# microsoft/fadtk

Measured on AMD Instinct MI355X. Metric: FAD scores/sec + cov-GEMM TFLOP/s (% MFMA peak), N=100k D=512, higher is better.
Workload: dtype f16 in, f16 MFMA with f32 accumulate over <= 8192-row runs, f64 across runs (moments); split-f16 MFMA iterations (f32 accumulate) + exact int8-MFMA products (int32 accumulate) + f64 correction (Frechet)

## Files before the change

### fadtk_amd/csrc/frechet.hip

```cpp
#include "frechet_internal.h"
#include "ns_mean.h"
#include "ns_fast.h"
#include "ns_fast_big.h"
#include "ns_fast_res.h"

#include <algorithm>
#include <atomic>
#include <cmath>
#include <type_traits>

namespace fad {

Pool& thread_pool(int device) {
    static thread_local PerThreadDevice<Pool> set;
    return set.get(device);
}
Workspace* free_slot(int device) {
    Pool& p = thread_pool(device);
    for (Workspace& w : p.slot)
        if (!w.busy) { w.pool = &p; return &w; }
    return nullptr;
}

SongKnobs SongKnobs::from_env() {
// ... 201 lines not shown
    }
    return f;
}

static int fast_prepare(Workspace& ws, int d, int ddof, const double* acc1, const double* acc2, const double* cov1, const double* cov2,
                        const double* mu1, const double* mu2, int mean_dtype, double* mus, double* covs, hipStream_t st,
                        const float* run1 = nullptr, const float* run2 = nullptr) {
    void* const before = ws.fast.p;
    FAD_TRY(ws.fast.reserve(fast_bytes(d)));
    FAD_TRY(ws.small.reserve(ns_small_bytes(d, 1)));
    FastBufs f = fast_bufs(ws, d);
    if (ws.fast.p != before) FAD_HIP_TRY(hipMemsetAsync(f.hdr, 0, 256, st));
    ws.job.gen = ++ws.fast_gen;
    if (ws.fast_gen > (1 << 30)) ws.fast_gen = 1;
    nsf::PrepArgs a;
    memset(&a, 0, sizeof(a));
    a.acc[0] = acc1; a.acc[1] = acc2; a.cov_in[0] = cov1; a.cov_in[1] = cov2; a.mu_in[0] = mu1; a.mu_in[1] = mu2;
    a.run[0] = run1; a.run[1] = run2;
    a.d = d; a.ddof = ddof; a.gen = ws.job.gen; a.mean_dtype = mean_dtype;
    a.mus = mus; a.covs = covs;
    a.dig[0] = f.digC[0]; a.dig[1] = f.digC[1];
    a.st = static_cast<NsState*>(ws.small.p);
    a.hdr[0] = f.hdr; a.hdr[1] = f.hdr + 1;
    hipLaunchKernelGGL(nsf::nsf_prepare, dim3((unsigned)((int64_t)d * d / 2048 + 1), 2), dim3(512), 0, st, a);
    FAD_HIP_TRY(hipGetLastError());
    return FAD_OK;
}

template <int NS> static void fast_launch_split(int mode, unsigned t, unsigned B, const nsf::SplitArgs& g, hipStream_t st) {
    if (mode == nsf::SP_FIRST) hipLaunchKernelGGL((nsf::nsf_split<NS, nsf::SP_FIRST>), dim3(t, t, B), dim3(512), 0, st, g);
    else if (mode == nsf::SP_T) hipLaunchKernelGGL((nsf::nsf_split<NS, nsf::SP_T>), dim3(t, t, B), dim3(512), 0, st, g);
    else if (mode == nsf::SP_V2) hipLaunchKernelGGL((nsf::nsf_split<NS, nsf::SP_V2>), dim3(t, t, 2 * B), dim3(512), 0, st, g);
    else if (mode == nsf::SP_V3) hipLaunchKernelGGL((nsf::nsf_split<NS, nsf::SP_V3>), dim3(t, t, B), dim3(512), 0, st, g);
    else hipLaunchKernelGGL((nsf::nsf_split<NS, nsf::SP_U>), dim3(t, t, 3 * B), dim3(512), 0, st, g);
}
static void fast_split(int d, int mode, const nsf::SplitArgs& g, hipStream_t st, unsigned B);
static void fast_verify_launch(int d, unsigned B, nsf::SplitArgs g, const nsf::SplitMat (&Y)[2], const nsf::SplitMat (&Z)[2], const nsf::SplitMat& Rv,
                               const nsf::SplitMat& Pv, const nsf::SplitMat& Ev, const Ns32State* s32, double* vstats, int* vwords, int64_t hstride,
                               hipStream_t st) {
    g.sel = &s32->final_iter; g.skip = &s32->skip_corr;
    g.Zf[0] = Z[0]; g.Zf[1] = Z[1]; g.Yf[0] = Y[0]; g.Yf[1] = Y[1];
    g.vstats = vstats; g.vwords = vwords; g.hstride = hstride;
    g.B[0] = Rv; g.C[0] = Pv; g.C[1] = Ev;
    fast_split(d, nsf::SP_V2, g, st, B);
    g.B[0] = Pv; g.A[1] = Ev; g.C[0] = nsf::SplitMat{nullptr, nullptr}; g.C[1] = nsf::SplitMat{nullptr, nullptr};
    fast_split(d, nsf::SP_V3, g, st, B);
}
static void fast_split(int d, int mode, const nsf::SplitArgs& g, hipStream_t st, unsigned B) {
    const unsigned t = (unsigned)(d / 32);
    switch (d) {
        case 128: fast_launch_split<1>(mode, t, B, g, st); break;
        case 256: fast_launch_split<2>(mode, t, B, g, st); break;
        case 384: fast_launch_split<3>(mode, t, B, g, st); break;
        case 512: fast_launch_split<4>(mode, t, B, g, st); break;
        case 768: fast_launch_split<6>(mode, t, B, g, st); break;
        default: fast_launch_split<8>(mode, t, B, g, st); break;
    }
}
template <int NJ> static void fast_big_attrs() {
    (void)hipFuncSetAttribute(reinterpret_cast<const void*>(&nsf::nsf_big<nsf::SP_T, NJ>), hipFuncAttributeMaxDynamicSharedMemorySize, (int)nsf::kBigLds);
    (void)hipFuncSetAttribute(reinterpret_cast<const void*>(&nsf::nsf_big<nsf::SP_U, NJ>), hipFuncAttributeMaxDynamicSharedMemorySize, (int)nsf::kBigLds);
    (void)hipFuncSetAttribute(reinterpret_cast<const void*>(&nsf::nsf_big<nsf::SP_FIRST, NJ>), hipFuncAttributeMaxDynamicSharedMemorySize, (int)nsf::kBigLds);
}
template <int NJ> static void fast_big_launch(int d, int mode, const nsf::SplitArgs& g, hipStream_t st, unsigned B) {
    const int tt = nsf::big_tiles(d, NJ);
    const unsigned one = (unsigned)nsf::big_grid((int)B, tt), two = (unsigned)nsf::big_grid((int)B, 2 * tt);
    if (mode == nsf::SP_FIRST) hipLaunchKernelGGL((nsf::nsf_big<nsf::SP_FIRST, NJ>), dim3(one), dim3(256), nsf::kBigLds, st, g);
    else if (mode == nsf::SP_T) hipLaunchKernelGGL((nsf::nsf_big<nsf::SP_T, NJ>), dim3(one), dim3(256), nsf::kBigLds, st, g);
    else hipLaunchKernelGGL((nsf::nsf_big<nsf::SP_U, NJ>), dim3(two + B), dim3(256), nsf::kBigLds, st, g);
}
static int fast_big_t_slots(int d, unsigned B) { return nsf::big_tiles(d, nsf::big_nj(d, 1, (int)B)); }
static int fast_split_big(int d, int mode, nsf::SplitArgs g, hipStream_t st, unsigned B, int device) {
    static std::atomic<unsigned> ready{0};
    if (device >= 0 && device < 32 && !(ready.load(std::memory_order_acquire) & (1u << device))) {
        fast_big_attrs<1>(); fast_big_attrs<2>();
        FAD_HIP_TRY(hipGetLastError());
        ready.fetch_or(1u << device, std::memory_order_release);
    }
    g.nprob = (int)B;
    if (nsf::big_nj(d, mode == nsf::SP_U ? 2 : 1, (int)B) == 1) fast_big_launch<1>(d, mode, g, st, B);
    else fast_big_launch<2>(d, mode, g, st, B);
    return FAD_OK;
}
static int fast_i8_big(int d, int mode, const nsf::I8Args& g, hipStream_t st, unsigned B, int device) {
    static std::atomic<unsigned> ready{0};
    if (device >= 0 && device < 32 && !(ready.load(std::memory_order_acquire) & (1u << device))) {
        FAD_HIP_TRY(hipFuncSetAttribute(reinterpret_cast<const void*>(&nsf::nsf_i8_big<nsf::I8_A>), hipFuncAttributeMaxDynamicSharedMemorySize, (int)nsf::kI8BigLds));
        FAD_HIP_TRY(hipFuncSetAttribute(reinterpret_cast<const void*>(&nsf::nsf_i8_big<nsf::I8_G>), hipFuncAttributeMaxDynamicSharedMemorySize, (int)nsf::kI8BigLds));
        FAD_HIP_TRY(hipFuncSetAttribute(reinterpret_cast<const void*>(&nsf::nsf_i8_big<nsf::I8_G, true>), hipFuncAttributeMaxDynamicSharedMemorySize, (int)nsf::kI8BigLds));
        ready.fetch_or(1u << device, std::memory_order_release);
    }
    const unsigned grid = (unsigned)nsf::big_grid((int)B, (d / 128) * (d / 64));
    if (mode == nsf::I8_A) hipLaunchKernelGGL((nsf::nsf_i8_big<nsf::I8_A>), dim3(grid), dim3(512), nsf::kI8BigLds, st, g, (int)B);
    else if (g.Rv.a) hipLaunchKernelGGL((nsf::nsf_i8_big<nsf::I8_G, true>), dim3(grid), dim3(512), nsf::kI8BigLds, st, g, (int)B);
    else hipLaunchKernelGGL((nsf::nsf_i8_big<nsf::I8_G>), dim3(grid), dim3(512), nsf::kI8BigLds, st, g, (int)B);
    return FAD_OK;
}
template <int NS8> static void fast_launch_i8(int mode, unsigned t, unsigned B, const nsf::I8Args& g, hipStream_t st) {
    if (mode == nsf::I8_A) hipLaunchKernelGGL((nsf::nsf_i8<NS8, nsf::I8_A>), dim3(t, t, B), dim3(512), 0, st, g);
    else hipLaunchKernelGGL((nsf::nsf_i8<NS8, nsf::I8_G>), dim3(t, t, B), dim3(512), 0, st, g);
}
static void fast_i8(int d, int mode, const nsf::I8Args& g, hipStream_t st, unsigned B = 1) {
    const unsigned t = (unsigned)(d / 32);
    switch (d) {
        case 128: case 256: fast_launch_i8<1>(mode, t, B, g, st); break;
        case 384: case 512: fast_launch_i8<2>(mode, t, B, g, st); break;
        case 768: fast_launch_i8<3>(mode, t, B, g, st); break;
        default: fast_launch_i8<4>(mode, t, B, g, st); break;
    }
}

static nsf::SplitArgs fast_split_args(Workspace& ws, const MixedBufs& m, const FastBufs& f, int d) {
    nsf::SplitArgs g;
    memset(&g, 0, sizeof(g));
    g.d = d; g.gen = ws.job.gen; g.hA = f.hdr; g.hB = f.hdr + 1; g.st = m.dstate; g.s32 = m.s32;
    if (wide_enabled(ws.pool)) { g.scaled = 1; g.lp_wide = 1; g.l0_scale = kWideL0Scale; g.l0_min = kWideL0Min; }
    return g;
}
static int fast_verify_enqueue(Workspace& ws) {
    const int d = ws.job.d;
    MixedBufs m = mixed_bufs(ws, d);
    FastBufs f = fast_bufs(ws, d);
    f.host_words[13] = 0;
    fast_verify_launch(d, 1, fast_split_args(ws, m, f, d), f.Y, f.Z, f.Rv, f.Pv, f.Ev, m.s32, f.host_vstats, f.host_words, 0, ws.job.stream);
    FAD_HIP_TRY(hipGetLastError());
    FAD_HIP_TRY(hipEventRecord(ws.done_ev, ws.job.stream));
    return FAD_OK;
}
static int fast_enqueue(Workspace& ws, int upto) {
    const int d = ws.job.d;
    hipStream_t stream = ws.job.stream;
    MixedBufs m = mixed_bufs(ws, d);
    FastBufs f = fast_bufs(ws, d);
    if (!f.host_words) return set_error(FAD_ERR_ALLOC, "pinned result area of the fast Frechet chain is missing");
    const int nslots = (d / 32) * (d / 32);
    const int max_low = max_low_of(ws);
    for (int& k = ws.job.k; k < upto; ++k) {
        nsf::SplitArgs g = fast_split_args(ws, m, f, d);
        if (k == 0) {
            nsf::I8Args a;
            memset(&a, 0, sizeof(a));
            a.Adig = f.digC[0]; a.Bdig = f.digC[1]; a.d = d; a.gen = ws.job.gen; a.hA = f.hdr; a.hB = f.hdr + 1; a.stats = m.tilestats;
            a.A64 = m.A; a.P = f.P; a.st = m.dstate;
            fast_i8(d, nsf::I8_A, a, stream);
            g.A[0] = f.P; g.B[0] = f.P; g.C[0] = f.Y[1]; g.C[1] = f.Z[1]; g.Cdig[0] = f.digY[1]; g.Cdig_t[0] = f.digYt[1];
            g.A64 = m.A; g.statsA = m.tilestats;
            fast_split(d, nsf::SP_FIRST, g, stream, 1);
            continue;
        }
        const int cur = k & 1;
        g.A[0] = f.Z[cur]; g.B[0] = f.Y[cur]; g.C[0] = f.T; g.alpha = -0.5f; g.beta_eye = 1.5f; g.gamma = 1.0f;
        g.partials = m.partials; g.skip = &m.s32->done; g.k = k;
        fast_split(d, nsf::SP_T, g, stream, 1);
        g = fast_split_args(ws, m, f, d);
        g.A[0] = f.Y[cur]; g.B[0] = f.T; g.C[0] = f.Y[cur ^ 1];
        g.A[1] = f.T; g.B[1] = f.Z[cur]; g.C[1] = f.Z[cur ^ 1];
        g.Cdig[0] = f.digY[cur ^ 1]; g.Cdig_t[0] = f.digYt[cur ^ 1];
        g.skip = &m.s32->upd_skip[k & 1];
        g.k = k; g.max_low = max_low; g.nslots = nslots; g.chk_partials = m.partials;
        g.thr_pred = pred_threshold(ws.pool, d);
        fast_split(d, nsf::SP_U, g, stream, 1);
    }
    nsf::I8Args a;
    memset(&a, 0, sizeof(a));
    a.Adig = f.digY[0]; a.Bdig = f.digYt[0]; a.Adig_alt = f.digY[1]; a.Bdig_alt = f.digYt[1]; a.sel = &m.s32->final_iter;
    a.d = d; a.gen = ws.job.gen; a.hA = f.hdr; a.hB = f.hdr + 1; a.skip = &m.s32->skip_corr; a.stats = f.host_stats; a.st = m.dstate; a.A64in = m.A;
    a.Y[0] = f.Y[0]; a.Y[1] = f.Y[1]; a.Z[0] = f.Z[0]; a.Z[1] = f.Z[1];
    a.s32 = m.s32; a.host_words = f.host_words; a.host_vals = f.host_vals;
    const bool wide = wide_enabled(ws.pool);
    if (wide) { a.Rv = f.Rv; a.scaled = 1; }
    f.host_words[12] = 0;
    f.host_words[13] = 0;
    fast_i8(d, nsf::I8_G, a, stream);
// ... 305 lines not shown
    const int nb = d / 32;
    int* h_words = reinterpret_cast<int*>(hpin + (nsf::kHostVals + (size_t)(nsf::kTileStats + 2) * nb * nb) * sizeof(double));
    double* h_vstats = reinterpret_cast<double*>(hpin + host_vstats_off(d));
    for (int b = 0; b < B; ++b) reinterpret_cast<int*>(reinterpret_cast<char*>(h_words) + (size_t)b * hs)[13] = 0;
    fast_verify_launch(d, (unsigned)B, g, Y, Z, mat(L.Rv), mat(L.Pv), mat(L.Ev), g.s32, h_vstats, h_words, (int64_t)hs, st);
    FAD_HIP_TRY(hipGetLastError());
    FAD_HIP_TRY(hipEventRecord(ws.done_ev, st));
    return FAD_OK;
}

static int pairs_enqueue(Workspace& ws, int d, int B, const fad_moments_t* const* h1, const fad_moments_t* const* h2, int ddof,
                         int mean_dtype, hipStream_t st) {
    const size_t dd = (size_t)d * d;
    const int nb = d / 32;
    constexpr int kPairsBigMin = 3;
    const bool big = B >= kPairsBigMin && d >= 256;
    const bool wide = wide_enabled(ws.pool);
    const int max_low = wide ? kMaxLowWide : kMaxLow;
    const int device = ws.job.device;
    const PairBlock L = pair_block(d);
    const size_t hs = song_host_stride(d);
    void* const before = ws.fast_pairs.p;
    FAD_TRY(ws.fast_pairs.reserve((size_t)(B > 16 ? kMaxMultiPairs : B > 8 ? 16 : B > 4 ? 8 : 4) * L.stride + 256));
    if (!ws.fast_pairs_pin || ws.fast_pairs_pin_cap < (size_t)B * hs) {
        if (ws.fast_pairs_pin) (void)hipHostFree(ws.fast_pairs_pin);
        ws.fast_pairs_pin = nullptr; ws.fast_pairs_pin_cap = 0;
        FAD_HIP_TRY(hipHostMalloc(&ws.fast_pairs_pin, (size_t)kMaxMultiPairs * hs + 4096, hipHostMallocDefault));
        ws.fast_pairs_pin_cap = (size_t)kMaxMultiPairs * hs + 4096;
    }
    char* blk = static_cast<char*>(ws.fast_pairs.p);
    char* hpin = static_cast<char*>(ws.fast_pairs_pin);
    double* h_vals = reinterpret_cast<double*>(hpin);
    double* h_stats = h_vals + nsf::kHostVals;
    int* h_words = reinterpret_cast<int*>(h_stats + (size_t)(nsf::kTileStats + 2) * nb * nb);
    auto at = [&](size_t off) { return blk + off; };
    auto mat = [&](size_t off) { nsf::SplitMat m; m.a = reinterpret_cast<uint4*>(at(off)); m.at = reinterpret_cast<uint4*>(at(off + 4 * dd)); return m; };
    const int gen = ++ws.fast_gen;
    if (ws.fast_gen > (1 << 30)) ws.fast_gen = 1;
    ws.multi.gen = gen;
    if (ws.fast_pairs.p != before) {
        FAD_HIP_TRY(hipMemset2DAsync(at(L.hdrA), L.stride, 0, sizeof(nsf::MatHdr), (size_t)B, st));
        FAD_HIP_TRY(hipMemset2DAsync(at(L.hdrB), L.stride, 0, sizeof(nsf::MatHdr), (size_t)B, st));
    }
    nsf::MatHdr* hA = reinterpret_cast<nsf::MatHdr*>(at(L.hdrA));
    nsf::MatHdr* hB = reinterpret_cast<nsf::MatHdr*>(at(L.hdrB));
    NsState* st0 = reinterpret_cast<NsState*>(at(L.st));
    Ns32State* s32_0 = reinterpret_cast<Ns32State*>(at(L.s32));
    double* partials = reinterpret_cast<double*>(at(L.partials));
    double* stats = reinterpret_cast<double*>(at(L.stats));
    double* A64 = reinterpret_cast<double*>(at(L.A64));
    const nsf::SplitMat P = mat(L.P), Y[2] = {mat(L.Y[0]), mat(L.Y[1])}, Z[2] = {mat(L.Z[0]), mat(L.Z[1])}, T = mat(L.T);
    uint4* digY[2] = {reinterpret_cast<uint4*>(at(L.digY[0])), reinterpret_cast<uint4*>(at(L.digY[1]))};
    uint4* digYt[2] = {reinterpret_cast<uint4*>(at(L.digYt[0])), reinterpret_cast<uint4*>(at(L.digYt[1]))};

    static_assert(2 * kMaxMultiPairs <= nsf::kPrepMaxSets, "PrepArgs holds two sets per pair of a batch");
    nsf::PrepArgs pa;
    memset(&pa, 0, sizeof(pa));
    for (int b = 0; b < B; ++b) {
        pa.accs[2 * b] = moments_packed(h1[b]); pa.accs[2 * b + 1] = moments_packed(h2[b]);
        pa.runs[2 * b] = moments_runsum(h1[b]); pa.runs[2 * b + 1] = moments_runsum(h2[b]);
    }
    pa.acc[0] = pa.accs[0]; pa.acc[1] = pa.accs[1];
    pa.d = d; pa.ddof = ddof; pa.gen = gen; pa.mean_dtype = mean_dtype;
    pa.mus = reinterpret_cast<double*>(at(L.mus)); pa.covs = reinterpret_cast<double*>(at(L.covs));
    pa.dig[0] = reinterpret_cast<uint4*>(at(L.digA)); pa.dig[1] = reinterpret_cast<uint4*>(at(L.digB));
    pa.st = st0; pa.hdr[0] = hA; pa.hdr[1] = hB;
    pa.batch = 2; pa.pstride = (int64_t)L.stride; pa.no_covs = 1;
    pa.per = ((dd / 2048) % 4 == 0) ? 4 : 2;
    hipLaunchKernelGGL(nsf::nsf_prepare, dim3((unsigned)(dd / 2048 / pa.per + 1), (unsigned)(2 * B)), dim3(512), 0, st, pa);

    auto split_args = [&]() {
        nsf::SplitArgs g;
        memset(&g, 0, sizeof(g));
        g.d = d; g.gen = gen; g.hA = hA; g.hB = hB; g.pstride = (int64_t)L.stride; g.astride = (int64_t)L.stride;
        g.st = st0; g.s32 = s32_0;
        if (wide) { g.scaled = 1; g.lp_wide = 1; g.l0_scale = kWideL0Scale; g.l0_min = kWideL0Min; }
        return g;
    };
    {
        nsf::I8Args a;
        memset(&a, 0, sizeof(a));
        a.Adig = reinterpret_cast<uint4*>(at(L.digA)); a.Bdig = reinterpret_cast<uint4*>(at(L.digB)); a.d = d; a.gen = gen; a.hA = hA; a.hB = hB;
        a.pstride = (int64_t)L.stride; a.astride = (int64_t)L.stride; a.stats = stats; a.A64 = A64; a.P = P; a.st = st0;
        if (big) FAD_TRY(fast_i8_big(d, nsf::I8_A, a, st, (unsigned)B, device));
        else fast_i8(d, nsf::I8_A, a, st, (unsigned)B);
        nsf::SplitArgs g = split_args();
        g.A[0] = P; g.B[0] = P; g.C[0] = Y[1]; g.C[1] = Z[1]; g.A64 = A64; g.statsA = stats;
        if (big) FAD_TRY(fast_split_big(d, nsf::SP_FIRST, g, st, (unsigned)B, device));
        else { g.Cdig[0] = digY[1]; g.Cdig_t[0] = digYt[1]; fast_split(d, nsf::SP_FIRST, g, st, (unsigned)B); }
    }
    int want = ws.pool ? ws.pool->lp_iters : 5;
    if (want < 2) want = 2;
    if (want > max_low) want = max_low;
    for (int k = 1; k < want; ++k) {
        const int cur = k & 1;
        nsf::SplitArgs g = split_args();
        g.A[0] = Z[cur]; g.B[0] = Y[cur]; g.C[0] = T; g.alpha = -0.5f; g.beta_eye = 1.5f; g.gamma = 1.0f;
        g.partials = partials; g.skip = &s32_0->done; g.k = k;
        if (big) FAD_TRY(fast_split_big(d, nsf::SP_T, g, st, (unsigned)B, device));
        else fast_split(d, nsf::SP_T, g, st, (unsigned)B);
        g = split_args();
        g.A[0] = Y[cur]; g.B[0] = T; g.C[0] = Y[cur ^ 1]; g.A[1] = T; g.B[1] = Z[cur]; g.C[1] = Z[cur ^ 1];
        if (!big) { g.Cdig[0] = digY[cur ^ 1]; g.Cdig_t[0] = digYt[cur ^ 1]; }
        g.skip = &s32_0->upd_skip[k & 1];
        g.k = k; g.max_low = max_low; g.nslots = big ? fast_big_t_slots(d, (unsigned)B) : nb * nb; g.chk_partials = partials; g.thr_pred = pred_threshold(ws.pool, d);
        if (big) FAD_TRY(fast_split_big(d, nsf::SP_U, g, st, (unsigned)B, device));
        else fast_split(d, nsf::SP_U, g, st, (unsigned)B);
    }
    if (big) {
        nsf::DigArgs dg;
        memset(&dg, 0, sizeof(dg));
        dg.d = d; dg.gen = gen; dg.hA = hA; dg.hB = hB; dg.pstride = (int64_t)L.stride; dg.astride = (int64_t)L.stride; dg.s32 = s32_0;
        dg.Y[0] = Y[0]; dg.Y[1] = Y[1]; dg.dig[0] = digY[0]; dg.dig[1] = digY[1]; dg.dig_t[0] = digYt[0]; dg.dig_t[1] = digYt[1];
        hipLaunchKernelGGL(nsf::nsf_digitize, dim3((unsigned)((dd / 16 + 255) / 256), 2, (unsigned)B), dim3(256), 0, st, dg);
    }
    {
        nsf::I8Args a;
        memset(&a, 0, sizeof(a));
        a.Adig = digY[0]; a.Bdig = digYt[0]; a.Adig_alt = digY[1]; a.Bdig_alt = digYt[1]; a.sel = &s32_0->final_iter;
        a.d = d; a.gen = gen; a.hA = hA; a.hB = hB; a.pstride = (int64_t)L.stride; a.astride = (int64_t)L.stride; a.hstride = (int64_t)hs;
        a.skip = &s32_0->skip_corr; a.stats = h_stats; a.st = st0; a.A64in = A64;
        a.Y[0] = Y[0]; a.Y[1] = Y[1]; a.Z[0] = Z[0]; a.Z[1] = Z[1]; a.s32 = s32_0; a.host_words = h_words; a.host_vals = h_vals;
        if (wide) { a.Rv = mat(L.Rv); a.scaled = 1; }
        for (int b = 0; b < B; ++b) { int* w = reinterpret_cast<int*>(reinterpret_cast<char*>(h_words) + (size_t)b * hs); w[12] = 0; w[13] = 0; }
        if (big) FAD_TRY(fast_i8_big(d, nsf::I8_G, a, st, (unsigned)B, device));
        else fast_i8(d, nsf::I8_G, a, st, (unsigned)B);
    }
    FAD_HIP_TRY(hipGetLastError());
    if (!ws.done_ev) FAD_HIP_TRY(hipEventCreateWithFlags(&ws.done_ev, hipEventDisableTiming));
    if (wide && ws.pool && ws.pool->lp_verify) return pairs_verify_enqueue(ws, d, B, st);
    FAD_HIP_TRY(hipEventRecord(ws.done_ev, st));
    return FAD_OK;
}

static int mixed_begin(const NsProblem& pb, int device, hipStream_t stream, Workspace& ws) {
    const int d = pb.d;
    const int64_t dd = (int64_t)d * d;
    FAD_TRY(ws.mats.reserve((size_t)(6 * dd) * sizeof(double)));
    FAD_TRY(ws.mats32.reserve((size_t)(5 * dd) * sizeof(float)));
    const size_t hbytes = ws.job.fast ? fast_pinned_bytes(d) : sizeof(NsState) + sizeof(MixedResult);
    if (!ws.pinned || ws.pinned_cap < hbytes) {
        if (ws.pinned) (void)hipHostFree(ws.pinned);
        ws.pinned = nullptr; ws.pinned_cap = 0;
        FAD_HIP_TRY(hipHostMalloc(&ws.pinned, hbytes + 4096, hipHostMallocDefault));
        ws.pinned_cap = hbytes + 4096;
    }
    MixedBufs m = mixed_bufs(ws, d);
    m.hres->status = -1;
    ws.job.d = d; ws.job.device = device; ws.job.stream = stream; ws.job.k = 0;
    if (ws.job.fast) {
        ws.job.mu1 = pb.mu1; ws.job.mu2 = pb.mu2; ws.job.mean_dtype = pb.mean_dtype;
        int want = ws.pool ? ws.pool->lp_iters : 5;
        if (want < 2) want = 2;
        if (want > max_low_of(ws)) want = max_low_of(ws);
        if (ws.pool && ws.pool->lp_hopeless) want = 1;
        return fast_enqueue(ws, want);
    }
    NsProductExt ext;
    memset(&ext, 0, sizeof(ext));
    ext.stats = m.tilestats; ext.mu1 = pb.mu1; ext.mu2 = pb.mu2; ext.mean_dtype = pb.mean_dtype; ext.st = m.dstate;
    FAD_TRY(gemm_f64_product_stats_launch(d, pb.cov1, pb.cov2, m.A, &m.dstate->done, ext, stream));
    enqueue_ns_prepare(m.tilestats, d, (int)m.nb, pb.mu1, 0, pb.mu2, 0, pb.mean_dtype, m.dstate, 1, m.s32, 1, stream);
    int want = ws.pool ? ws.pool->lp_iters : 5;
    if (want < 2) want = 2;
    if (want > kMaxLow) want = kMaxLow;
    return mixed_enqueue(ws, want);
}

static int mixed_finish(Workspace& ws, MixedResult* res) {
    MixedBufs m = mixed_bufs(ws, ws.job.d);
    const int max_low = max_low_of(ws);
    bool asked = false;
    for (;;) {
        FAD_HIP_TRY(hipEventSynchronize(ws.done_ev));
        if (ws.job.fast) FAD_TRY(fast_decide(ws));
        if (m.hres->status == 5) {
            if (asked) { m.hres->status = 2; break; }
            asked = true;
            FAD_TRY(fast_verify_enqueue(ws));
            continue;
        }
        if (m.hres->status == 4) {
            ws.job.k = m.hres->iters;
            m.hres->status = 0;
        } else if (m.hres->status != 0 || ws.job.k >= max_low) {
            break;
        }
        if (ws.job.k >= max_low) break;
        const int step = (ws.job.fast && max_low > kMaxLow) ? 4 : 2;
        const int upto = (ws.job.k + step < max_low) ? ws.job.k + step : max_low;
        FAD_TRY(ws.job.fast ? fast_enqueue(ws, upto) : mixed_enqueue(ws, upto));
    }
    *res = *m.hres;
    if (res->status == 0) res->status = 2;
    if (res->status == 1 && res->decided_at >= 0 && ws.pool) ws.pool->lp_iters = res->decided_at + 1;
    if (ws.pool && ws.job.fast) {
        ws.pool->lp_hopeless = res->status == 2 && res->iters < 0;
        ws.pool->lp_verify = res->status == 1 && res->pad == 1;
    }
    return FAD_OK;
}

static bool mixed_eligible(Workspace& ws, int d, int max_iter, double tol) {
    Pool* p = ws.pool;
    if (p && p->mixed < 0) { const char* e = getenv("FAD_FRECHET_MIXED"); p->mixed = (e && e[0] == '0') ? 0 : 1; }
    return (!p || p->mixed) && d % 64 == 0 && max_iter <= 0 && tol <= 0.0;
}

// ... 353 lines not shown
```

### fadtk_amd/csrc/ns_fast_big.h

```cpp
#pragma once
#include "ns_fast.h"
#include "big_slots.h"

namespace fad {
namespace nsf {

#ifndef FAD_BIG_STAGES
#define FAD_BIG_STAGES 3
#endif
constexpr int kBigStages = FAD_BIG_STAGES;
constexpr int kBigStage = 1024;
constexpr size_t kBigLds = (size_t)kBigStages * kBigStage * 16 + 256;

template <int MODE, int NJ = 2>
__global__ __launch_bounds__(256, (FAD_BIG_STAGES <= 3) ? 3 : ((FAD_BIG_STAGES <= 4) ? 2 : 1)) void nsf_big(SplitArgs g) {
    static_assert(MODE == SP_T || MODE == SP_U || MODE == SP_FIRST, "SP_FIRST: iteration 0 (scale from nsf_i8<A>'s statistics, Y1, Z1)");
    extern __shared__ __attribute__((aligned(16))) uint4 ring[];
    double* red = reinterpret_cast<double*>(ring + kBigStages * kBigStage);
    const int d = g.d, tid = threadIdx.x, lane = tid & 63;
    constexpr int ZP = (MODE == SP_U) ? 2 : 1;
    const int t = d >> 7, tx_n = (NJ == 2) ? t : 2 * t, tt = t * tx_n;
    const int L = blockIdx.x;
    const int nprod = big_grid(g.nprob, tt * ZP);
    if constexpr (MODE == SP_U) {
// ... 139 lines not shown
#pragma unroll
        for (int j = 0; j < NJ; ++j) { bh[j] = st[(8 + (NJ * wc + j) * 2) * 64]; bl[j] = st[(8 + (NJ * wc + j) * 2 + 1) * 64]; }
#pragma unroll
        for (int i = 0; i < 2; ++i)
#pragma unroll
            for (int j = 0; j < NJ; ++j) {
                acc0[i][j] = __builtin_amdgcn_mfma_f32_32x32x16_f16(ah[i], bh[j], acc0[i][j], 0, 0, 0);
                acc1[i][j] = __builtin_amdgcn_mfma_f32_32x32x16_f16(ah[i], bl[j], acc1[i][j], 0, 0, 0);
                acc1[i][j] = __builtin_amdgcn_mfma_f32_32x32x16_f16(al[i], bh[j], acc1[i][j], 0, 0, 0);
            }
    }
    __syncthreads();
#ifdef FAD_BIG_ABL_NOEPI
    if (acc0[0][0][0] != 12345.678f) return;
#endif

    float* fin = reinterpret_cast<float*>(ring) + wave * (32 * 33 + 32);
    const int kg = lane >> 5, r = lane & 31;
    float alpha = (MODE == SP_T) ? g.alpha : 1.f, beta = (MODE == SP_T) ? g.beta_eye : 0.f, gamma = g.gamma;
    if (MODE == SP_T && g.scaled) {
        const double m = adv(g.st, po)->mu[g.k];
        alpha = (float)(-0.5 * m * m * m); beta = (float)(1.5 * m); gamma = beta + alpha;
    }
    const SplitMat Cm = adv(g.C[zi], po);
    const bool with_digits = (MODE == SP_U) && zi == 0 && g.Cdig[0];
    uint4* dig = with_digits ? adv(g.Cdig[0], po) : nullptr;
    uint4* dig_t = with_digits ? adv(g.Cdig_t[0], po) : nullptr;
    double ss = 0.0;
#pragma unroll
    for (int i = 0; i < 2; ++i)
#pragma unroll
        for (int j = 0; j < NJ; ++j) {
            const int by = 4 * TY + 2 * wr + i, bx = 2 * NJ * TX + NJ * wc + j;
            if constexpr (MODE == SP_FIRST) {
                const double* A64 = adv(g.A64, po) + (int64_t)(32 * by + 4 * kg) * d + 32 * bx + r;
                float z1[16];
#pragma unroll
                for (int reg = 0; reg < 16; ++reg) {
                    const int q = (reg & 3) + 8 * (reg >> 2);
                    const float y0 = (float)(A64[(int64_t)q * d] * inv_c);
                    const float y2 = (float)((double)(acc0[i][j][reg] + acc1[i][j][reg] * kLoInv) * (inv_cn * inv_cn));
                    fin[(q + 4 * kg) * 33 + r] = m1 * y0 - m3 * y2;
                    z1[reg] = ((by == bx && q + 4 * kg == r) ? m1 : 0.f) - m3 * y0;
                }
                __builtin_amdgcn_wave_barrier();
#pragma unroll
                for (int pass = 0; pass < 4; ++pass) store_tile_planes(fin, Cm, by, bx, d, pass * 64 + lane);
                __builtin_amdgcn_wave_barrier();
#pragma unroll
                for (int reg = 0; reg < 16; ++reg) fin[((reg & 3) + 8 * (reg >> 2) + 4 * kg) * 33 + r] = z1[reg];
                __builtin_amdgcn_wave_barrier();
                const SplitMat Zm1 = adv(g.C[1], po);
#pragma unroll
                for (int pass = 0; pass < 4; ++pass) store_tile_planes(fin, Zm1, by, bx, d, pass * 64 + lane);
                __builtin_amdgcn_wave_barrier();
                continue;
            }
            float ssf = 0.f;
#pragma unroll
            for (int reg = 0; reg < 16; ++reg) {
                const int q = (reg & 3) + 8 * (reg >> 2) + 4 * kg;
                const bool dg = (by == bx) && (q == r);
                const float v = alpha * (acc0[i][j][reg] + acc1[i][j][reg] * kLoInv) + (dg ? beta : 0.f);
                if constexpr (MODE == SP_T) { const float e = v - (dg ? gamma : 0.f); ssf = __builtin_fmaf(e, e, ssf); }
                fin[q * 33 + r] = v;
            }
            ss += (double)ssf;
            __builtin_amdgcn_wave_barrier();
#pragma unroll
            for (int pass = 0; pass < 4; ++pass) store_tile_planes(fin, Cm, by, bx, d, pass * 64 + lane);
            if (with_digits) {
#pragma unroll 2
                for (int pass = 0; pass < 8; ++pass) store_tile_digits(fin, dig, dig_t, by, bx, d, pass * 64 + lane);
            }
            __builtin_amdgcn_wave_barrier();
        }
    if constexpr (MODE == SP_T) {
        double s1[1] = {ss};
        wg8_sum<1, 4>(s1, red);
        if (tid == 0) adv(g.partials, po)[tile] = s1[0];
    }
}

constexpr int kI8BigStage = 36 * 64;
#ifndef FAD_I8_BIG_STAGES
#define FAD_I8_BIG_STAGES 2
#endif
constexpr int kI8BigStages = FAD_I8_BIG_STAGES;
constexpr size_t kI8BigLds = (size_t)kI8BigStages * kI8BigStage * 16 + 256;

template <int MODE, bool WITHR = false>
__global__ __launch_bounds__(512) void nsf_i8_big(I8Args g, int nprob) {
    extern __shared__ __attribute__((aligned(16))) uint4 ring[];
    double* red = reinterpret_cast<double*>(ring + kI8BigStages * kI8BigStage);
    constexpr int kUmin = (MODE == I8_A) ? kUminA : kUminG;
    constexpr int kGroups = 2 * (kDigits - 1) - kUmin + 1;
    const int d = g.d, tid = threadIdx.x, lane = tid & 63;
    const int tr_ = d >> 7, tc_ = d >> 6, tt = tr_ * tc_;
    const BigSlot slot = big_slot(blockIdx.x, nprob, tt);
    if (!slot.live) return;
    const int song = slot.song, tile = slot.item;
    const int TY = tile / tc_, TX = tile - TY * tc_;
    const int64_t po = (int64_t)song * g.pstride, ho = (int64_t)song * g.hstride;
    const MatHdr* hB = adv(g.hB, po);
    const MatHdr* hA = adv(g.hA, (int64_t)song * g.astride);
    NsState* const st_p = adv(g.st, po);
    const bool bad = hdr_bad(hA, hB, g.gen);
    const bool skipped = bad || (g.skip && *adv(g.skip, po) != 0);
    if constexpr (MODE == I8_G) {
        if (tile == 0 && tid == 0) {
            const NsState* st = st_p; const Ns32State* s = adv(g.s32, po);
            int* hw = adv(g.host_words, ho); double* hv = adv(g.host_vals, ho);
            hw[0] = bad ? 1 : 0; hw[1] = st->done; hw[2] = st->nonfinite; hw[3] = st->too_few[0]; hw[4] = st->too_few[1];
            hw[5] = s->ok; hw[6] = s->failed; hw[7] = s->final_iter; hw[8] = s->decided_at; hw[9] = s->strict; hw[10] = s->finished;
            hw[11] = skipped ? 1 : 0;
            hv[0] = st->c; hv[1] = st->tr1; hv[2] = st->tr2; hv[3] = st->mean_term;
#pragma unroll
            for (int q = 0; q < 16; ++q) hv[4 + q] = s->res[q];
            hw[14] = (g.scaled && st->mu[0] != 1.0) ? 1 : 0;
            hw[12] = g.gen;
        }
    }
    if (skipped) return;
    const int wave = __builtin_amdgcn_readfirstlane(tid >> 6);
    const int wr = wave >> 1, wc = wave & 1;
    const bool alt = (MODE == I8_G) && g.sel && (*adv(g.sel, po) & 1);
    const uint4* Ad = (MODE == I8_A) ? adv(g.Adig, (int64_t)song * g.astride) : adv(alt ? g.Adig_alt : g.Adig, po);
    const uint4* Bd = adv(alt ? g.Bdig_alt : g.Bdig, po);
#ifdef FAD_I8_ABL_G_NOLOOP
    const int nks = (MODE == I8_G) ? 0 : (d >> 5);
#else
    const int nks = d >> 5;
#endif

    const uint32_t voff = (uint32_t)lane * 16u;
    const uint32_t ring_lds = (uint32_t)(size_t)(__attribute__((address_space(3))) void*)ring;
    auto issue = [&](int ks) {
#pragma unroll
        for (int i = 0; i < 5; ++i) {
            const int q = wave + 8 * i;
            if (q < 36) {
                const bool bs = q >= 24;
                const int blk = bs ? (q - 24) / 6 : q / 6, p = bs ? (q - 24) % 6 : q % 6;
                const uint64_t sb = (uint64_t)((bs ? Bd : Ad) + dg_idx((bs ? 2 * TX : 4 * TY) + blk, ks, p, 0, d));
                const uint32_t lo = __builtin_amdgcn_readfirstlane((uint32_t)sb);
                const uint32_t hi = __builtin_amdgcn_readfirstlane((uint32_t)(sb >> 32));
                const uint64_t ub = ((uint64_t)hi << 32) | lo;
                const uint32_t m0v = __builtin_amdgcn_readfirstlane(ring_lds + (uint32_t)(((ks % kI8BigStages) * kI8BigStage + q * 64) * 16));
                asm volatile("s_mov_b32 m0, %2\n\ts_nop 0\n\tglobal_load_lds_dwordx4 %0, %1" ::"v"(voff), "s"(ub), "s"(m0v) : "memory", "m0");
            }
        }
    };
    i32x16 acc[kGroups];
#pragma unroll
    for (int u = 0; u < kGroups; ++u)
#pragma unroll
        for (int q = 0; q < 16; ++q) acc[u][q] = 0;
    static_assert(kI8BigStages >= 2 && kI8BigStages <= 4, "the counted waits below cover two younger stages at most");
    for (int ks = 0; ks < kI8BigStages - 1 && ks < nks; ++ks) issue(ks);
    const bool five = wave < 4;
    for (int ks = 0; ks < nks; ++ks) {
        const int ahead = (nks - 1 - ks < kI8BigStages - 2) ? (nks - 1 - ks) : (kI8BigStages - 2);
        if (ahead == 2) { if (five) asm volatile("s_waitcnt vmcnt(10)" ::: "memory"); else asm volatile("s_waitcnt vmcnt(8)" ::: "memory"); }
        else if (ahead == 1) { if (five) asm volatile("s_waitcnt vmcnt(5)" ::: "memory"); else asm volatile("s_waitcnt vmcnt(4)" ::: "memory"); }
        else asm volatile("s_waitcnt vmcnt(0)" ::: "memory");
        __builtin_amdgcn_s_barrier();
#ifndef FAD_I8_ABL_NODMA
        if (ks + kI8BigStages - 1 < nks) issue(ks + kI8BigStages - 1);
#endif
        const i32x4* st = reinterpret_cast<const i32x4*>(ring + (ks % kI8BigStages) * kI8BigStage) + lane;
        i32x4 a[kDigits], b[kDigits];
#pragma unroll
        for (int p = 0; p < kDigits; ++p) { a[p] = st[(wr * 6 + p) * 64]; b[p] = st[(24 + wc * 6 + p) * 64]; }
#ifdef FAD_I8_ABL_NOMMA
#pragma unroll
        for (int p = 0; p < kDigits; ++p) { acc[0][p] += a[p][0] ^ b[p][1]; acc[1][p] += a[p][2] ^ b[p][3]; }
#else
#pragma unroll
        for (int p = kDigits - 1; p >= 0; --p)
#pragma unroll
            for (int q = kDigits - 1; q >= 0; --q)
                if (p + q >= kUmin) acc[p + q - kUmin] = __builtin_amdgcn_mfma_i32_32x32x32_i8(a[p], b[q], acc[p + q - kUmin], 0, 0, 0);
#endif
    }
    __syncthreads();
    double gp[16];
#pragma unroll
    for (int q = 0; q < 16; ++q) gp[q] = 0.0;
#pragma unroll
    for (int u = 0; u < kGroups; ++u) {
        const double wgt = __builtin_ldexp(1.0, 7 * (u + kUmin) - 80);
#pragma unroll
        for (int q = 0; q < 16; ++q) gp[q] = __builtin_fma((double)acc[u][q], wgt, gp[q]);
    }
    float* fin = reinterpret_cast<float*>(ring) + wave * (32 * 33 + 32);
    const int kg = lane >> 5, n = lane & 31;
    const int by = 4 * TY + wr, bx = 2 * TX + wc, nb = d >> 5;
    const int row0 = 32 * by, col0 = 32 * bx;
    double* const stats = adv(g.stats, (MODE == I8_A) ? po : ho);
    double* scal = stats + (size_t)kTileStats * (by * nb + bx);
    double v3[3] = {0.0, 0.0, 0.0};
    if constexpr (MODE == I8_A) {
        const double inv = hdr_inv_s12(hA, hB);
        double* A64 = adv(g.A64, po) + (int64_t)(row0 + 4 * kg) * d + col0 + n;
#pragma unroll
        for (int reg = 0; reg < 16; ++reg) {
            const int q = (reg & 3) + 8 * (reg >> 2);
            A64[(int64_t)q * d] = gp[reg] * inv;
            fin[(q + 4 * kg) * 33 + n] = (float)gp[reg];
            v3[0] += gp[reg] * gp[reg];
            if (by == bx && q + 4 * kg == n) v3[1] += gp[reg];
        }
        __builtin_amdgcn_wave_barrier();
        const SplitMat Pm = adv(g.P, po);
#pragma unroll
        for (int pass = 0; pass < 4; ++pass) store_tile_planes(fin, Pm, by, bx, d, pass * 64 + lane);
    } else {
        const SplitMat Zm = adv(g.Z[alt ? 1 : 0], po);
        const SplitMat Ym = adv(g.Y[alt ? 1 : 0], po);
        const double inv_c = 1.0 / st_p->c;
        const double* A64 = adv(g.A64in, po) + (int64_t)(row0 + 4 * kg) * d + col0 + n;
        typedef _Float16 f16x4 __attribute__((ext_vector_type(4)));
        f16x4 zh[4], zl[4];
#pragma unroll
        for (int j = 0; j < 4; ++j) {
            int half;
            const size_t zi = fa_elem(col0 + n, row0 + 8 * j + 4 * kg, 0, d, half);
            zh[j] = *reinterpret_cast<const f16x4*>(reinterpret_cast<const _Float16*>(Zm.a + zi) + half);
            zl[j] = *reinterpret_cast<const f16x4*>(reinterpret_cast<const _Float16*>(Zm.a + zi + 64) + half);
        }
#pragma unroll
        for (int reg = 0; reg < 16; ++reg) {
            const int q = (reg & 3) + 8 * (reg >> 2), gr = row0 + q + 4 * kg, gc = col0 + n;
            const double R = A64[(int64_t)q * d] * inv_c - gp[reg];
            if constexpr (WITHR) gp[reg] = R;
            const double z = (double)used16(zh[reg >> 2][reg & 3], zl[reg >> 2][reg & 3]);
            v3[0] += z * R; v3[1] += R * R;
            if (by == bx && gr == gc) {
                int hy;
                const size_t yi = fa_elem(gr, gr, 0, d, hy);
                v3[2] += (double)used16(reinterpret_cast<const _Float16*>(Ym.a + yi)[hy], reinterpret_cast<const _Float16*>(Ym.a + yi + 64)[hy]);
            }
            fin[(q + 4 * kg) * 33 + n] = fabsf((float)z);
        }
        __builtin_amdgcn_wave_barrier();
    }
    double m = 0.0;
    if constexpr (MODE == I8_A) {
        if (lane < 32) { for (int c = 0; c < 32; ++c) m += fabsf(fin[lane * 33 + c]); }
        else { for (int q = 0; q < 32; ++q) m += fabsf(fin[q * 33 + lane - 32]); }
    } else {
        if (lane < 32) { for (int q = 0; q < 32; ++q) m += fin[q * 33 + lane]; }
        else { for (int c = 0; c < 32; ++c) m += fin[(lane - 32) * 33 + c]; }
    }
    double mrow = (lane < 32) ? m : 0.0, mcol = (lane >= 32) ? m : 0.0;
#pragma unroll
    for (int off = 32; off > 0; off >>= 1) {
        mrow = fmax(mrow, __shfl_xor(mrow, off)); mcol = fmax(mcol, __shfl_xor(mcol, off));
#pragma unroll
        for (int q = 0; q < 3; ++q) v3[q] += __shfl_xor(v3[q], off);
    }
    if (lane == 0) {
        if constexpr (MODE == I8_A) {
            scal[0] = v3[0]; scal[1] = v3[1]; scal[2] = mrow; scal[3] = mcol;
        } else {
            scal[0] = v3[0]; scal[1] = v3[1]; scal[2] = v3[2]; scal[3] = 0.0;
            double* zmax = stats + (size_t)kTileStats * nb * nb + 2 * (size_t)(by * nb + bx);
            zmax[0] = mrow; zmax[1] = mcol;
        }
    }
    if constexpr (MODE == I8_G && WITHR) {
        if (g.Rv.a) {
            __builtin_amdgcn_wave_barrier();
#pragma unroll
            for (int reg = 0; reg < 16; ++reg) fin[((reg & 3) + 8 * (reg >> 2) + 4 * kg) * 33 + n] = (float)(gp[reg] * (double)kVerScale);
            __builtin_amdgcn_wave_barrier();
            const SplitMat Rm = adv(g.Rv, po);
#pragma unroll
            for (int pass = 0; pass < 4; ++pass) store_tile_planes(fin, Rm, by, bx, d, pass * 64 + lane);
        }
    }
    (void)red;
}

}
}
```

Measured before the change: 12650.

## Add 2x2-wave int8 MFMA tile kernel for big Frechet path and trim epilogue registers

Turns the big int8-MFMA product kernel into a template parameterised by its wave grid. It adds a 64x64-tile, 256-thread variant (nsf_i8_quad, launch bounds allowing 3 blocks per CU) that both I8_A and I8_G now use on the big path. The epilogue computes f64 partial sums per register on demand instead of holding a 16-double array, and it loads Z in two halves, to cut register pressure. This gives more blocks and more occupancy, but the smaller tiles reload digit operands more often and lower per-block reuse.

After: 12490. 1.2% lower.

```diff
diff --git a/fadtk_amd/csrc/frechet.hip b/fadtk_amd/csrc/frechet.hip
--- a/fadtk_amd/csrc/frechet.hip
+++ b/fadtk_amd/csrc/frechet.hip
@@ -307,13 +307,23 @@
     else fast_big_launch<2>(d, mode, g, st, B);
     return FAD_OK;
 }
-static int fast_i8_big(int d, int mode, const nsf::I8Args& g, hipStream_t st, unsigned B, int device) {
+static int fast_i8_big(int d, int mode, const nsf::I8Args& g, hipStream_t st, unsigned B, int device, bool quad = false) {
     static std::atomic<unsigned> ready{0};
     if (device >= 0 && device < 32 && !(ready.load(std::memory_order_acquire) & (1u << device))) {
         FAD_HIP_TRY(hipFuncSetAttribute(reinterpret_cast<const void*>(&nsf::nsf_i8_big<nsf::I8_A>), hipFuncAttributeMaxDynamicSharedMemorySize, (int)nsf::kI8BigLds));
         FAD_HIP_TRY(hipFuncSetAttribute(reinterpret_cast<const void*>(&nsf::nsf_i8_big<nsf::I8_G>), hipFuncAttributeMaxDynamicSharedMemorySize, (int)nsf::kI8BigLds));
         FAD_HIP_TRY(hipFuncSetAttribute(reinterpret_cast<const void*>(&nsf::nsf_i8_big<nsf::I8_G, true>), hipFuncAttributeMaxDynamicSharedMemorySize, (int)nsf::kI8BigLds));
+        FAD_HIP_TRY(hipFuncSetAttribute(reinterpret_cast<const void*>(&nsf::nsf_i8_quad<nsf::I8_A>), hipFuncAttributeMaxDynamicSharedMemorySize, (int)nsf::kI8QuadLds));
+        FAD_HIP_TRY(hipFuncSetAttribute(reinterpret_cast<const void*>(&nsf::nsf_i8_quad<nsf::I8_G>), hipFuncAttributeMaxDynamicSharedMemorySize, (int)nsf::kI8QuadLds));
+        FAD_HIP_TRY(hipFuncSetAttribute(reinterpret_cast<const void*>(&nsf::nsf_i8_quad<nsf::I8_G, true>), hipFuncAttributeMaxDynamicSharedMemorySize, (int)nsf::kI8QuadLds));
         ready.fetch_or(1u << device, std::memory_order_release);
+    }
+    if (quad) {
+        const unsigned grid = (unsigned)nsf::big_grid((int)B, nsf::i8_quad_tiles(d));
+        if (mode == nsf::I8_A) hipLaunchKernelGGL((nsf::nsf_i8_quad<nsf::I8_A>), dim3(grid), dim3(256), nsf::kI8QuadLds, st, g, (int)B);
+        else if (g.Rv.a) hipLaunchKernelGGL((nsf::nsf_i8_quad<nsf::I8_G, true>), dim3(grid), dim3(256), nsf::kI8QuadLds, st, g, (int)B);
+        else hipLaunchKernelGGL((nsf::nsf_i8_quad<nsf::I8_G>), dim3(grid), dim3(256), nsf::kI8QuadLds, st, g, (int)B);
+        return FAD_OK;
     }
     const unsigned grid = (unsigned)nsf::big_grid((int)B, (d / 128) * (d / 64));
     if (mode == nsf::I8_A) hipLaunchKernelGGL((nsf::nsf_i8_big<nsf::I8_A>), dim3(grid), dim3(512), nsf::kI8BigLds, st, g, (int)B);
@@ -785,7 +795,7 @@
         memset(&a, 0, sizeof(a));
         a.Adig = reinterpret_cast<uint4*>(at(L.digA)); a.Bdig = reinterpret_cast<uint4*>(at(L.digB)); a.d = d; a.gen = gen; a.hA = hA; a.hB = hB;
         a.pstride = (int64_t)L.stride; a.astride = (int64_t)L.stride; a.stats = stats; a.A64 = A64; a.P = P; a.st = st0;
-        if (big) FAD_TRY(fast_i8_big(d, nsf::I8_A, a, st, (unsigned)B, device));
+        if (big) FAD_TRY(fast_i8_big(d, nsf::I8_A, a, st, (unsigned)B, device, true));
         else fast_i8(d, nsf::I8_A, a, st, (unsigned)B);
         nsf::SplitArgs g = split_args();
         g.A[0] = P; g.B[0] = P; g.C[0] = Y[1]; g.C[1] = Z[1]; g.A64 = A64; g.statsA = stats;
@@ -826,7 +836,7 @@
         a.Y[0] = Y[0]; a.Y[1] = Y[1]; a.Z[0] = Z[0]; a.Z[1] = Z[1]; a.s32 = s32_0; a.host_words = h_words; a.host_vals = h_vals;
         if (wide) { a.Rv = mat(L.Rv); a.scaled = 1; }
         for (int b = 0; b < B; ++b) { int* w = reinterpret_cast<int*>(reinterpret_cast<char*>(h_words) + (size_t)b * hs); w[12] = 0; w[13] = 0; }
-        if (big) FAD_TRY(fast_i8_big(d, nsf::I8_G, a, st, (unsigned)B, device));
+        if (big) FAD_TRY(fast_i8_big(d, nsf::I8_G, a, st, (unsigned)B, device, true));
         else fast_i8(d, nsf::I8_G, a, st, (unsigned)B);
     }
     FAD_HIP_TRY(hipGetLastError());
diff --git a/fadtk_amd/csrc/ns_fast_big.h b/fadtk_amd/csrc/ns_fast_big.h
--- a/fadtk_amd/csrc/ns_fast_big.h
+++ b/fadtk_amd/csrc/ns_fast_big.h
@@ -245,21 +245,24 @@
     }
 }
 
-constexpr int kI8BigStage = 36 * 64;
 #ifndef FAD_I8_BIG_STAGES
 #define FAD_I8_BIG_STAGES 2
 #endif
 constexpr int kI8BigStages = FAD_I8_BIG_STAGES;
+constexpr int i8_tile_stage(int WR, int WC) { return (WR + WC) * kDigits * 64; }
+constexpr int kI8BigStage = i8_tile_stage(4, 2), kI8QuadStage = i8_tile_stage(2, 2);
 constexpr size_t kI8BigLds = (size_t)kI8BigStages * kI8BigStage * 16 + 256;
-
-template <int MODE, bool WITHR = false>
-__global__ __launch_bounds__(512) void nsf_i8_big(I8Args g, int nprob) {
-    extern __shared__ __attribute__((aligned(16))) uint4 ring[];
-    double* red = reinterpret_cast<double*>(ring + kI8BigStages * kI8BigStage);
+constexpr size_t kI8QuadLds = (size_t)kI8BigStages * kI8QuadStage * 16 + 256;
+constexpr int i8_quad_tiles(int d) { return (d / 64) * (d / 64); }
+
+template <int MODE, bool WITHR, int WR, int WC>
+__device__ __forceinline__ void i8_tile(const I8Args& g, int nprob, uint4* ring) {
+    constexpr int NW = WR * WC, kStage = i8_tile_stage(WR, WC), kPieces = kStage / 64, kPerWave = (kPieces + NW - 1) / NW;
     constexpr int kUmin = (MODE == I8_A) ? kUminA : kUminG;
     constexpr int kGroups = 2 * (kDigits - 1) - kUmin + 1;
+    static_assert(NW * (32 * 33 + 32) * 4 <= kI8BigStages * kStage * 16, "the epilogue's float areas live in the ring");
     const int d = g.d, tid = threadIdx.x, lane = tid & 63;
-    const int tr_ = d >> 7, tc_ = d >> 6, tt = tr_ * tc_;
+    const int tr_ = d / (32 * WR), tc_ = d / (32 * WC), tt = tr_ * tc_;
     const BigSlot slot = big_slot(blockIdx.x, nprob, tt);
     if (!slot.live) return;
     const int song = slot.song, tile = slot.item;
@@ -286,7 +289,7 @@
     }
     if (skipped) return;
     const int wave = __builtin_amdgcn_readfirstlane(tid >> 6);
-    const int wr = wave >> 1, wc = wave & 1;
+    const int wr = wave / WC, wc = wave % WC;
     const bool alt = (MODE == I8_G) && g.sel && (*adv(g.sel, po) & 1);
     const uint4* Ad = (MODE == I8_A) ? adv(g.Adig, (int64_t)song * g.astride) : adv(alt ? g.Adig_alt : g.Adig, po);
     const uint4* Bd = adv(alt ? g.Bdig_alt : g.Bdig, po);
@@ -300,16 +303,16 @@
     const uint32_t ring_lds = (uint32_t)(size_t)(__attribute__((address_space(3))) void*)ring;
     auto issue = [&](int ks) {
 #pragma unroll
-        for (int i = 0; i < 5; ++i) {
-            const int q = wave + 8 * i;
-            if (q < 36) {
-                const bool bs = q >= 24;
-                const int blk = bs ? (q - 24) / 6 : q / 6, p = bs ? (q - 24) % 6 : q % 6;
-                const uint64_t sb = (uint64_t)((bs ? Bd : Ad) + dg_idx((bs ? 2 * TX : 4 * TY) + blk, ks, p, 0, d));
+        for (int i = 0; i < kPerWave; ++i) {
+            const int q = wave + NW * i;
+            if (q < kPieces) {
+                const bool bs = q >= 6 * WR;
+                const int blk = bs ? (q - 6 * WR) / 6 : q / 6, p = bs ? (q - 6 * WR) % 6 : q % 6;
+                const uint64_t sb = (uint64_t)((bs ? Bd : Ad) + dg_idx((bs ? WC * TX : WR * TY) + blk, ks, p, 0, d));
                 const uint32_t lo = __builtin_amdgcn_readfirstlane((uint32_t)sb);
                 const uint32_t hi = __builtin_amdgcn_readfirstlane((uint32_t)(sb >> 32));
                 const uint64_t ub = ((uint64_t)hi << 32) | lo;
-                const uint32_t m0v = __builtin_amdgcn_readfirstlane(ring_lds + (uint32_t)(((ks % kI8BigStages) * kI8BigStage + q * 64) * 16));
+                const uint32_t m0v = __builtin_amdgcn_readfirstlane(ring_lds + (uint32_t)(((ks % kI8BigStages) * kStage + q * 64) * 16));
                 asm volatile("s_mov_b32 m0, %2\n\ts_nop 0\n\tglobal_load_lds_dwordx4 %0, %1" ::"v"(voff), "s"(ub), "s"(m0v) : "memory", "m0");
             }
         }
@@ -321,20 +324,20 @@
         for (int q = 0; q < 16; ++q) acc[u][q] = 0;
     static_assert(kI8BigStages >= 2 && kI8BigStages <= 4, "the counted waits below cover two younger stages at most");
     for (int ks = 0; ks < kI8BigStages - 1 && ks < nks; ++ks) issue(ks);
-    const bool five = wave < 4;
+    const bool full = (kPieces % NW == 0) || wave < kPieces % NW;
     for (int ks = 0; ks < nks; ++ks) {
         const int ahead = (nks - 1 - ks < kI8BigStages - 2) ? (nks - 1 - ks) : (kI8BigStages - 2);
-        if (ahead == 2) { if (five) asm volatile("s_waitcnt vmcnt(10)" ::: "memory"); else asm volatile("s_waitcnt vmcnt(8)" ::: "memory"); }
-        else if (ahead == 1) { if (five) asm volatile("s_waitcnt vmcnt(5)" ::: "memory"); else asm volatile("s_waitcnt vmcnt(4)" ::: "memory"); }
+        if (ahead == 2) { if (full) asm volatile("s_waitcnt vmcnt(%0)" ::"n"(2 * kPerWave) : "memory"); else asm volatile("s_waitcnt vmcnt(%0)" ::"n"(2 * kPerWave - 2) : "memory"); }
+        else if (ahead == 1) { if (full) asm volatile("s_waitcnt vmcnt(%0)" ::"n"(kPerWave) : "memory"); else asm volatile("s_waitcnt vmcnt(%0)" ::"n"(kPerWave - 1) : "memory"); }
         else asm volatile("s_waitcnt vmcnt(0)" ::: "memory");
         __builtin_amdgcn_s_barrier();
 #ifndef FAD_I8_ABL_NODMA
         if (ks + kI8BigStages - 1 < nks) issue(ks + kI8BigStages - 1);
 #endif
-        const i32x4* st = reinterpret_cast<const i32x4*>(ring + (ks % kI8BigStages) * kI8BigStage) + lane;
+        const i32x4* st = reinterpret_cast<const i32x4*>(ring + (ks % kI8BigStages) * kStage) + lane;
         i32x4 a[kDigits], b[kDigits];
 #pragma unroll
-        for (int p = 0; p < kDigits; ++p) { a[p] = st[(wr * 6 + p) * 64]; b[p] = st[(24 + wc * 6 + p) * 64]; }
+        for (int p = 0; p < kDigits; ++p) { a[p] = st[(wr * 6 + p) * 64]; b[p] = st[(6 * WR + wc * 6 + p) * 64]; }
 #ifdef FAD_I8_ABL_NOMMA
 #pragma unroll
         for (int p = 0; p < kDigits; ++p) { acc[0][p] += a[p][0] ^ b[p][1]; acc[1][p] += a[p][2] ^ b[p][3]; }
@@ -347,32 +350,31 @@
 #endif
     }
     __syncthreads();
-    double gp[16];
-#pragma unroll
-    for (int q = 0; q < 16; ++q) gp[q] = 0.0;
-#pragma unroll
-    for (int u = 0; u < kGroups; ++u) {
-        const double wgt = __builtin_ldexp(1.0, 7 * (u + kUmin) - 80);
-#pragma unroll
-        for (int q = 0; q < 16; ++q) gp[q] = __builtin_fma((double)acc[u][q], wgt, gp[q]);
-    }
+    auto gp_of = [&](int reg) {
+        double v = 0.0;
+#pragma unroll
+        for (int u = 0; u < kGroups; ++u) v = __builtin_fma((double)acc[u][reg], __builtin_ldexp(1.0, 7 * (u + kUmin) - 80), v);
+        return v;
+    };
     float* fin = reinterpret_cast<float*>(ring) + wave * (32 * 33 + 32);
     const int kg = lane >> 5, n = lane & 31;
-    const int by = 4 * TY + wr, bx = 2 * TX + wc, nb = d >> 5;
+    const int by = WR * TY + wr, bx = WC * TX + wc, nb = d >> 5;
     const int row0 = 32 * by, col0 = 32 * bx;
     double* const stats = adv(g.stats, (MODE == I8_A) ? po : ho);
     double* scal = stats + (size_t)kTileStats * (by * nb + bx);
     double v3[3] = {0.0, 0.0, 0.0};
+    float rv[WITHR ? 16 : 1];
     if constexpr (MODE == I8_A) {
         const double inv = hdr_inv_s12(hA, hB);
         double* A64 = adv(g.A64, po) + (int64_t)(row0 + 4 * kg) * d + col0 + n;
 #pragma unroll
         for (int reg = 0; reg < 16; ++reg) {
             const int q = (reg & 3) + 8 * (reg >> 2);
-            A64[(int64_t)q * d] = gp[reg] * inv;
-            fin[(q + 4 * kg) * 33 + n] = (float)gp[reg];
-            v3[0] += gp[reg] * gp[reg];
-            if (by == bx && q + 4 * kg == n) v3[1] += gp[reg];
+            const double gp = gp_of(reg);
+            A64[(int64_t)q * d] = gp * inv;
+            fin[(q + 4 * kg) * 33 + n] = (float)gp;
+            v3[0] += gp * gp;
+            if (by == bx && q + 4 * kg == n) v3[1] += gp;
         }
         __builtin_amdgcn_wave_barrier();
         const SplitMat Pm = adv(g.P, po);
@@ -384,27 +386,30 @@
         const double inv_c = 1.0 / st_p->c;
         const double* A64 = adv(g.A64in, po) + (int64_t)(row0 + 4 * kg) * d + col0 + n;
         typedef _Float16 f16x4 __attribute__((ext_vector_type(4)));
-        f16x4 zh[4], zl[4];
-#pragma unroll
-        for (int j = 0; j < 4; ++j) {
-            int half;
-            const size_t zi = fa_elem(col0 + n, row0 + 8 * j + 4 * kg, 0, d, half);
-            zh[j] = *reinterpret_cast<const f16x4*>(reinterpret_cast<const _Float16*>(Zm.a + zi) + half);
-            zl[j] = *reinterpret_cast<const f16x4*>(reinterpret_cast<const _Float16*>(Zm.a + zi + 64) + half);
-        }
-#pragma unroll
-        for (int reg = 0; reg < 16; ++reg) {
-            const int q = (reg & 3) + 8 * (reg >> 2), gr = row0 + q + 4 * kg, gc = col0 + n;
-            const double R = A64[(int64_t)q * d] * inv_c - gp[reg];
-            if constexpr (WITHR) gp[reg] = R;
-            const double z = (double)used16(zh[reg >> 2][reg & 3], zl[reg >> 2][reg & 3]);
-            v3[0] += z * R; v3[1] += R * R;
-            if (by == bx && gr == gc) {
-                int hy;
-                const size_t yi = fa_elem(gr, gr, 0, d, hy);
-                v3[2] += (double)used16(reinterpret_cast<const _Float16*>(Ym.a + yi)[hy], reinterpret_cast<const _Float16*>(Ym.a + yi + 64)[hy]);
-            }
-            fin[(q + 4 * kg) * 33 + n] = fabsf((float)z);
+#pragma unroll
+        for (int h = 0; h < 2; ++h) {
+            f16x4 zh[2], zl[2];
+#pragma unroll
+            for (int j = 0; j < 2; ++j) {
+                int half;
+                const size_t zi = fa_elem(col0 + n, row0 + 8 * (2 * h + j) + 4 * kg, 0, d, half);
+                zh[j] = *reinterpret_cast<const f16x4*>(reinterpret_cast<const _Float16*>(Zm.a + zi) + half);
+                zl[j] = *reinterpret_cast<const f16x4*>(reinterpret_cast<const _Float16*>(Zm.a + zi + 64) + half);
+            }
+#pragma unroll
+            for (int reg = 8 * h; reg < 8 * h + 8; ++reg) {
+                const int q = (reg & 3) + 8 * (reg >> 2), gr = row0 + q + 4 * kg, gc = col0 + n;
+                const double R = A64[(int64_t)q * d] * inv_c - gp_of(reg);
+                if constexpr (WITHR) rv[reg] = (float)(R * (double)kVerScale);
+                const double z = (double)used16(zh[(reg >> 2) & 1][reg & 3], zl[(reg >> 2) & 1][reg & 3]);
+                v3[0] += z * R; v3[1] += R * R;
+                if (by == bx && gr == gc) {
+                    int hy;
+                    const size_t yi = fa_elem(gr, gr, 0, d, hy);
+                    v3[2] += (double)used16(reinterpret_cast<const _Float16*>(Ym.a + yi)[hy], reinterpret_cast<const _Float16*>(Ym.a + yi + 64)[hy]);
+                }
+                fin[(q + 4 * kg) * 33 + n] = fabsf((float)z);
+            }
         }
         __builtin_amdgcn_wave_barrier();
     }
@@ -436,15 +441,25 @@
         if (g.Rv.a) {
             __builtin_amdgcn_wave_barrier();
 #pragma unroll
-            for (int reg = 0; reg < 16; ++reg) fin[((reg & 3) + 8 * (reg >> 2) + 4 * kg) * 33 + n] = (float)(gp[reg] * (double)kVerScale);
+            for (int reg = 0; reg < 16; ++reg) fin[((reg & 3) + 8 * (reg >> 2) + 4 * kg) * 33 + n] = rv[reg];
             __builtin_amdgcn_wave_barrier();
             const SplitMat Rm = adv(g.Rv, po);
 #pragma unroll
             for (int pass = 0; pass < 4; ++pass) store_tile_planes(fin, Rm, by, bx, d, pass * 64 + lane);
         }
     }
-    (void)red;
-}
-
-}
-}
+}
+
+template <int MODE, bool WITHR = false>
+__global__ __launch_bounds__(512) void nsf_i8_big(I8Args g, int nprob) {
+    extern __shared__ __attribute__((aligned(16))) uint4 ring[];
+    i8_tile<MODE, WITHR, 4, 2>(g, nprob, ring);
+}
+template <int MODE, bool WITHR = false>
+__global__ __launch_bounds__(256, 3) void nsf_i8_quad(I8Args g, int nprob) {
+    extern __shared__ __attribute__((aligned(16))) uint4 ring[];
+    i8_tile<MODE, WITHR, 2, 2>(g, nprob, ring);
+}
+
+}
+}
```
